# lambdaclass/AES_zero_knowledge_proof_circuit

Hardware: AMD Instinct MI355X
Metric: AES-ECB blocks proven/sec (Marlin), proof verifies (higher is better)
Workload: dtype u32 limbs (253-bit Fr / 377-bit Fq modular integers)

## Files before the change

aes_zero_knowledge_proof_circuit_amd/csrc/ff28.cuh:

```cuda
#pragma once
#include "ff.cuh"

namespace zk {

template <class P>
struct Fp28 {
    static constexpr int N = 14;
    static constexpr uint32_t MASK = (1u << 28) - 1;
    uint32_t l[N];

    ZK_HD static constexpr uint32_t mod28(int i) {
        int bit = 28 * i, w = bit >> 5, sh = bit & 31;
        uint64_t two = (w < P::N ? (uint64_t)P::mod(w) : 0) | ((w + 1 < P::N ? (uint64_t)P::mod(w + 1) : 0) << 32);
        return (uint32_t)(two >> sh) & MASK;
    }
    static constexpr uint32_t PINV = P::INV & MASK;

    ZK_HD static Fp28 zero() { Fp28 r; for (int i = 0; i < N; i++) r.l[i] = 0; return r; }
    ZK_HD bool limbs_zero() const { uint32_t o = 0; for (int i = 0; i < N; i++) o |= l[i]; return o == 0; }
    ZK_HD static bool product_is_zero(const Fp28 &v) {
        if (v.l[0] != 0u && v.l[0] != mod28(0)) return false;
        uint32_t z0 = 0, zp = 0;
#pragma unroll
        for (int i = 0; i < N; i++) { z0 |= v.l[i]; zp |= v.l[i] ^ mod28(i); }
        return z0 == 0 || zp == 0;
    }

    ZK_HD static Fp28 split(const uint32_t *w) {
        Fp28 r;
#pragma unroll
        for (int i = 0; i < N; i++) {
            int bit = 28 * i, k = bit >> 5, sh = bit & 31;
            uint64_t two = (k < P::N ? (uint64_t)w[k] : 0) | ((k + 1 < P::N ? (uint64_t)w[k + 1] : 0) << 32);
            r.l[i] = (uint32_t)(two >> sh) & MASK;
        }
        return r;
    }
    ZK_HD void pack(uint32_t *w) const {
#pragma unroll
        for (int k = 0; k < P::N; k++) {
            int bit = 32 * k, i = bit / 28, sh = bit % 28;
            uint64_t v = (uint64_t)l[i] >> sh;
            int have = 28 - sh;
            if (i + 1 < N) v |= (uint64_t)l[i + 1] << have;
            if (have + 28 < 32 && i + 2 < N) v |= (uint64_t)l[i + 2] << (have + 28);
            w[k] = (uint32_t)v;
        }
    }
    ZK_HD static Fp28 normalize(const int64_t *t) {
        Fp28 r;
        int64_t c = 0;
#pragma unroll
        for (int i = 0; i < N - 1; i++) { int64_t v = t[i] + c; r.l[i] = (uint32_t)v & MASK; c = v >> 28; }
        r.l[N - 1] = (uint32_t)(t[N - 1] + c);
        return r;
    }
    ZK_HD Fp28 operator+(const Fp28 &b) const {
        Fp28 r;
        uint32_t c = 0;
#pragma unroll
        for (int i = 0; i < N - 1; i++) { uint32_t v = l[i] + b.l[i] + c; r.l[i] = v & MASK; c = v >> 28; }
        r.l[N - 1] = l[N - 1] + b.l[N - 1] + c;
        return r;
    }
    ZK_HD Fp28 dbl() const { return *this + *this; }
    ZK_HD Fp28 add_lazy(const Fp28 &b) const { Fp28 r; for (int i = 0; i < N; i++) r.l[i] = l[i] + b.l[i]; return r; }
    ZK_HD Fp28 dbl_lazy() const { Fp28 r; for (int i = 0; i < N; i++) r.l[i] = l[i] << 1; return r; }
    template <int K> ZK_HD Fp28 sub_lazy(const Fp28 &b) const {
        Fp28 r;
#pragma unroll
        for (int i = 0; i < N; i++) {
#if defined(__HIP_DEVICE_COMPILE__)
            if (i < N - 1) { asm("v_sad_u32 %0, %1, %2, %3" : "=v"(r.l[i]) : "s"(kp_spread<K>(i)), "v"(b.l[i]), "v"(l[i])); continue; }
#endif
            r.l[i] = l[i] + kp_spread<K>(i) - b.l[i];
        }
        return r;
    }
    template <int K> ZK_HD static constexpr uint32_t kp_limb(int i) {
        uint64_t c = 0, v = 0;
        for (int j = 0; j <= i; j++) { v = (uint64_t)K * mod28(j) + c; c = v >> 28; }
        return i == N - 1 ? (uint32_t)v : (uint32_t)v & MASK;
    }
    template <int K> ZK_HD static constexpr uint32_t kp_spread(int i) {
        return i == 0 ? kp_limb<K>(0) + (1u << 28) : (i == N - 1 ? kp_limb<K>(i) - 1u : kp_limb<K>(i) + MASK);
    }
    template <int K>
    ZK_HD Fp28 sub(const Fp28 &b) const {
        Fp28 r;
        uint32_t c = 0;
#pragma unroll
        for (int i = 0; i < N - 1; i++) { uint32_t v = l[i] + kp_spread<K>(i) - b.l[i] + c; r.l[i] = v & MASK; c = v >> 28; }
        r.l[N - 1] = l[N - 1] + kp_spread<K>(N - 1) - b.l[N - 1] + c;
        return r;
    }

    ZK_HD static void reduce_row(uint64_t *t, int i) {
        if constexpr (mod28(0) == 1u && PINV == MASK) {
            const uint64_t u = t[i] + MASK;
            const uint32_t m = ~(uint32_t)u & MASK;
#pragma unroll
            for (int j = 1; j < N; j++) t[i + j] += (uint64_t)m * mod28(j);
            t[i + 1] += u >> 28;
        } else {
            uint32_t m = (((uint32_t)t[i] & MASK) * PINV) & MASK;
#pragma unroll
            for (int j = 0; j < N; j++) t[i + j] += (uint64_t)m * mod28(j);
            t[i + 1] += t[i] >> 28;
        }
    }

    ZK_HD Fp28 operator*(const Fp28 &b) const {
        uint64_t t[2 * N];
#pragma unroll
        for (int i = 0; i < 2 * N; i++) t[i] = 0;
#pragma unroll
        for (int i = 0; i < N; i++) {
#pragma unroll
            for (int j = 0; j < N; j++) t[i + j] += (uint64_t)l[j] * b.l[i];
            reduce_row(t, i);
        }
        Fp28 r;
        uint64_t c = 0;
#pragma unroll
        for (int i = 0; i < N - 1; i++) { uint64_t v = t[N + i] + c; r.l[i] = (uint32_t)v & MASK; c = v >> 28; }
        r.l[N - 1] = (uint32_t)(t[2 * N - 1] + c);
        return r;
    }
    ZK_HD static Fp28 mul_biased(const Fp28 &a, const Fp28 &b, uint64_t bias) {
        static_assert(mod28(0) == 1u && PINV == MASK, "written for p = 1 (mod 2^28)");
        uint64_t t[2 * N];
#pragma unroll
        for (int i = 0; i < 2 * N; i++) t[i] = i < N ? bias : 0;
#pragma unroll
        for (int i = 0; i < N; i++) {
#pragma unroll
            for (int j = 0; j < N; j++) t[i + j] += (uint64_t)a.l[j] * b.l[i];
            const uint64_t u = t[i];
            const uint32_t m = ~(uint32_t)u & MASK;
#pragma unroll
            for (int j = 1; j < N; j++) t[i + j] += (uint64_t)m * mod28(j);
            t[i + 1] += u >> 28;
        }
        Fp28 r;
        uint64_t c = 0;
#pragma unroll
        for (int i = 0; i < N - 1; i++) { uint64_t v = t[N + i] + c; r.l[i] = (uint32_t)v & MASK; c = v >> 28; }
        r.l[N - 1] = (uint32_t)(t[2 * N - 1] + c);
        return r;
    }
    ZK_HD static uint64_t hot_loop_bias() {
        uint64_t v = MASK;
#if defined(__HIP_DEVICE_COMPILE__)
        asm volatile("" : "+s"(v));
#endif
        return v;
    }
    ZK_HD static Fp28 fma2(const Fp28 &a, const Fp28 &b, const Fp28 &c, const Fp28 &d) {
        uint64_t t[2 * N];
#pragma unroll
        for (int i = 0; i < 2 * N; i++) t[i] = 0;
#pragma unroll
        for (int i = 0; i < N; i++) {
#pragma unroll
            for (int j = 0; j < N; j++) t[i + j] += (uint64_t)a.l[j] * b.l[i];
#pragma unroll
            for (int j = 0; j < N; j++) t[i + j] += (uint64_t)c.l[j] * d.l[i];
            reduce_row(t, i);
        }
        Fp28 r;
        uint64_t cy = 0;
#pragma unroll
        for (int i = 0; i < N - 1; i++) { uint64_t v = t[N + i] + cy; r.l[i] = (uint32_t)v & MASK; cy = v >> 28; }
        r.l[N - 1] = (uint32_t)(t[2 * N - 1] + cy);
        return r;
    }
    ZK_HD Fp28 sqr() const {
        uint64_t t[2 * N];
#pragma unroll
        for (int i = 0; i < 2 * N; i++) t[i] = 0;
        uint32_t d[N];
#pragma unroll
        for (int i = 0; i < N; i++) d[i] = l[i] << 1;
#pragma unroll
        for (int i = 0; i < N; i++) {
            t[2 * i] += (uint64_t)l[i] * l[i];
#pragma unroll
            for (int j = i + 1; j < N; j++) t[i + j] += (uint64_t)d[i] * l[j];
        }
#pragma unroll
        for (int i = 0; i < N; i++) {
            reduce_row(t, i);
        }
        Fp28 r;
        uint64_t c = 0;
#pragma unroll
        for (int i = 0; i < N - 1; i++) { uint64_t v = t[N + i] + c; r.l[i] = (uint32_t)v & MASK; c = v >> 28; }
        r.l[N - 1] = (uint32_t)(t[2 * N - 1] + c);
        return r;
    }

    ZK_HD Fp28 canonical() const {
        Fp28 v = *this;
#pragma unroll
        for (int k = 5; k >= 0; k--) {
            int64_t c = 0;
            uint32_t tl[N];
#pragma unroll
            for (int i = 0; i < N - 1; i++) { int64_t x = (int64_t)v.l[i] - ((int64_t)mod28(i) << k) + c; tl[i] = (uint32_t)x & MASK; c = x >> 28; }
            int64_t top = (int64_t)v.l[N - 1] - ((int64_t)mod28(N - 1) << k) + c;
            if (top >= 0) {
#pragma unroll
                for (int i = 0; i < N - 1; i++) v.l[i] = tl[i];
                v.l[N - 1] = (uint32_t)top;
            }
        }
        return v;
    }
    ZK_HD bool is_zero_mod_p() const { return canonical().limbs_zero(); }

    ZK_HD static Fp28 from_std(const Fp<P> &a) {
        Fp28 s = split(a.l);
        return s * k_2_400();
    }
    ZK_HD Fp<P> to_std() const {
        Fp28 y = (*this * k_2_384()).canonical();
        Fp<P> r;
        y.pack(r.l);
        return r;
    }
    ZK_HD static Fp28 k_2_384() { Fp<P> o = Fp<P>::one(); return split(o.l); }
    ZK_HD static Fp28 k_one() { return k_2_392(); }
    ZK_HD static Fp28 k_2_392() {
        Fp<P> v = Fp<P>::one();
        for (int i = 0; i < 8; i++) v = v.dbl();
        return split(v.l);
    }
    ZK_HD static Fp28 k_2_400() {
        Fp<P> v = Fp<P>::one();
        for (int i = 0; i < 16; i++) v = v.dbl();
        return split(v.l);
    }
};

using Fq377x28 = Fp28<Fq377P>;
using Fq381x28 = Fp28<Fq381P>;

}
```

aes_zero_knowledge_proof_circuit_amd/csrc/te28.cuh:

```cuda
#pragma once
#include "ec28.cuh"

namespace zk {

template <class P>
struct alignas(64) Niels28 { FpMsm<P> ymx, ypx, td; uint32_t pad[6]; };
template <class P>
struct AccTE { FpMsm<P> x, y, z, t; };

struct Te377 {
    using P = Fq377P;
    using G = Fp28<P>;
    using F = Fp<P>;
    ZK_HD static G lit28(const uint32_t (&t)[14]) { G r; for (int i = 0; i < 14; i++) r.l[i] = t[i]; return r; }
    ZK_HD static F lit(const uint32_t (&t)[12]) { F r; for (int i = 0; i < 12; i++) r.l[i] = t[i]; return r; }
    ZK_HD static F s_std() { constexpr uint32_t t[12] = FQ377_TE_S_INIT; return lit(t); }
    ZK_HD static F f_std() { constexpr uint32_t t[12] = FQ377_TE_F_INIT; return lit(t); }
    ZK_HD static F k2d_std() { constexpr uint32_t t[12] = FQ377_TE_K2D_INIT; return lit(t); }
    ZK_HD static G k2d() { constexpr uint32_t t[14] = FQ377_TE_K2D_28_INIT; return lit28(t); }
    ZK_HD static G si() { constexpr uint32_t t[14] = FQ377_TE_SI_28_INIT; return lit28(t); }
    ZK_HD static G sif() { constexpr uint32_t t[14] = FQ377_TE_SIF_28_INIT; return lit28(t); }
};

template <class P>
ZK_HD AccTE<P> te_identity() { AccTE<P> r; r.x = FpMsm<P>::zero(); r.t = r.x; r.y = FpMsm<P>::k_one(); r.z = r.y; return r; }
template <class P>
ZK_HD Niels28<P> niels_identity() { Niels28<P> r; r.ymx = FpMsm<P>::k_one(); r.ypx = r.ymx; r.td = FpMsm<P>::zero(); return r; }
template <class P>
ZK_HD Niels28<P> niels_neg(const Niels28<P> &n) { Niels28<P> r; r.ymx = n.ypx; r.ypx = n.ymx; r.td = FpMsm<P>::zero().template sub<2>(n.td); return r; }

template <class P>
ZK_HD void te_madd(AccTE<P> &a, const Niels28<P> &n) {
    using G = FpMsm<P>;
    G A = a.y.template sub_lazy<3>(a.x) * n.ymx;
    G B = a.y.add_lazy(a.x) * n.ypx;
    G C = a.t * n.td;
    G D = a.z.dbl_lazy();
    G E = B.template sub<2>(A), H = B.add_lazy(A);
    G F = D.template sub_lazy<2>(C), Gg = D + C;
    a.x = E * F; a.y = Gg * H; a.t = E * H; a.z = F * Gg;
}
template <class P>
ZK_HD Niels28<P> niels_load_signed(const Niels28<P> *rec, bool neg) {
    const FpMsm<P> *f = &rec->ymx;
    Niels28<P> r;
    r.ymx = f[neg ? 1 : 0]; r.ypx = f[neg ? 0 : 1]; r.td = rec->td;
    return r;
}
template <class P>
ZK_HD void te_madd_hot(AccTE<P> &a, Niels28<P> &n, bool neg, const Niels28<P> *next, bool next_neg, uint64_t bias) {
    using G = FpMsm<P>;
    G A = G::mul_biased(a.y.template sub_lazy<3>(a.x), n.ymx, bias);
    G B = G::mul_biased(a.y.add_lazy(a.x), n.ypx, bias);
    G C = G::mul_biased(a.t, n.td, bias);
#if defined(__HIP_DEVICE_COMPILE__)
    asm volatile("" : "+v"(A.l[G::N - 1]), "+v"(B.l[G::N - 1]), "+v"(C.l[G::N - 1]) : : "memory");
#endif
    n = niels_load_signed<P>(next, next_neg);
#if defined(__HIP_DEVICE_COMPILE__)
    asm volatile("" : "+v"(A.l[0]), "+v"(C.l[0]) : : "memory");
#endif
    G E = B.template sub_lazy<2>(A), H = B.add_lazy(A);
    G D = a.z.dbl_lazy();
    G U = D.template sub_lazy<2>(C), V = D.add_lazy(C), F, Gg;
#pragma unroll
    for (int i = 0; i < G::N; i++) { F.l[i] = neg ? V.l[i] : U.l[i]; Gg.l[i] = neg ? U.l[i] : V.l[i]; }
    a.x = G::mul_biased(E, F, bias); a.y = G::mul_biased(Gg, H, bias); a.t = G::mul_biased(E, H, bias); a.z = G::mul_biased(F, Gg, bias);
}
template <class P>
ZK_HD void te_add_inline(AccTE<P> &a, const AccTE<P> &b) {
    using G = FpMsm<P>;
    G A = a.y.template sub<3>(a.x) * b.y.template sub<3>(b.x);
    G B = (a.y + a.x) * (b.y + b.x);
    G C = (a.t * b.t) * Te377::k2d();
    G D = (a.z * b.z).dbl();
    G E = B.template sub<2>(A), H = B + A;
    G F = D.template sub<2>(C), Gg = D + C;
    a.x = E * F; a.y = Gg * H; a.t = E * H; a.z = F * Gg;
}
template <class P>
ZK_EC_FN void te_add(AccTE<P> &a, const AccTE<P> &b) { te_add_inline<P>(a, b); }
template <class P>
ZK_EC_FN void te_dbl(AccTE<P> &a) {
    using G = FpMsm<P>;
    G A = a.x.sqr(), B = a.y.sqr(), C = a.z.sqr().dbl();
    G S = (a.x + a.y).sqr(), AB = A + B;
    G E = S.template sub<3>(AB);
    G Gg = B.template sub<2>(A);
    G F = Gg.template sub<3>(C);
    G H = G::zero().template sub<3>(AB);
    a.x = E * F; a.y = Gg * H; a.t = E * H; a.z = F * Gg;
}
template <class P>
ZK_HD AccTE<P> te_neg(const AccTE<P> &a) {
    AccTE<P> r = a;
    if (!a.x.limbs_zero()) r.x = FpMsm<P>::zero().template sub<2>(a.x);
    if (!a.t.limbs_zero()) r.t = FpMsm<P>::zero().template sub<2>(a.t);
    return r;
}

template <class P>
ZK_HD XYZZ<Fp<P>> te_to_std_point(const AccTE<P> &a) {
    using G = FpMsm<P>;
    G zmy = a.z.template sub<3>(a.y), zpy = a.z + a.y;
    G xz = a.x * zmy;
    G zz = xz.sqr();
    if (zz.is_zero_mod_p()) return XYZZ<Fp<P>>::inf();
    G numx = (Te377::si() * zpy).template sub<6>(zmy);
    XYZZ<Fp<P>> o;
    o.x = ((numx * a.x) * xz).to_std();
    o.y = (((Te377::sif() * a.z) * zpy) * zz).to_std();
    o.zz = zz.to_std();
    o.zzz = (zz * xz).to_std();
    return o;
}

struct TeMapParts { Fp<Fq377P> u, v, den; };
ZK_HD TeMapParts te_map_parts(const Affine<Fp<Fq377P>> &p) {
    using F = Fp<Fq377P>;
    TeMapParts m;
    F s = Te377::s_std();
    m.u = s * (p.x + F::one());
    m.v = s * p.y;
    m.den = m.v * (m.u + F::one());
    return m;
}
ZK_HD Niels28<Fq377P> te_niels_finish(const TeMapParts &m, const Fp<Fq377P> &den_inv) {
    using F = Fp<Fq377P>;
    using G = FpMsm<Fq377P>;
    F xe = Te377::f_std() * m.u * (m.u + F::one()) * den_inv;
    F ye = (m.u - F::one()) * m.v * den_inv;
    Niels28<Fq377P> n;
    n.ymx = G::from_std(ye - xe);
    n.ypx = G::from_std(ye + xe);
    n.td = G::from_std(Te377::k2d_std() * xe * ye);
    return n;
}
ZK_HD Niels28<Fq377P> niels_from_weierstrass(const Affine<Fp<Fq377P>> &p, bool *bad) {
    if (p.is_inf()) return niels_identity<Fq377P>();
    TeMapParts m = te_map_parts(p);
    if (m.den.is_zero()) { if (bad) *bad = true; return niels_identity<Fq377P>(); }
    return te_niels_finish(m, m.den.inverse());
}

#if defined(__HIPCC__)
template <int CTRL> __device__ __forceinline__ uint32_t quad_dpp(uint32_t v) {
#if defined(__HIP_DEVICE_COMPILE__)
    return (uint32_t)__builtin_amdgcn_mov_dpp((int)v, CTRL, 0xf, 0xf, true);
#else
    return v;
#endif
}
template <int CTRL, class G> __device__ __forceinline__ G quad_move(const G &v) {
    G r;
#pragma unroll
    for (int i = 0; i < G::N; i++) r.l[i] = quad_dpp<CTRL>(v.l[i]);
    return r;
}
constexpr int QP_LANE0 = 0x00, QP_LANE1 = 0x55, QP_LANE2 = 0xAA, QP_LANE3 = 0xFF, QP_SWAP_PAIRS = 0xB1;
template <class G> __device__ __forceinline__ G quad_pick(int q, const G &v0, const G &v1, const G &v2, const G &v3) {
    G r;
#pragma unroll
    for (int i = 0; i < G::N; i++) r.l[i] = q == 0 ? v0.l[i] : (q == 1 ? v1.l[i] : (q == 2 ? v2.l[i] : v3.l[i]));
    return r;
}
template <class P>
__device__ __forceinline__ FpMsm<P> te_quad_finish(int q, const FpMsm<P> &E, const FpMsm<P> &F, const FpMsm<P> &Gg, const FpMsm<P> &H) {
    return quad_pick(q, E, Gg, F, E) * quad_pick(q, F, H, Gg, H);
}
template <class P>
__device__ __forceinline__ FpMsm<P> te_add_quad(const FpMsm<P> &a, const FpMsm<P> &b, int q) {
    using G = FpMsm<P>;
    const G oa = quad_move<QP_SWAP_PAIRS>(a), ob = quad_move<QP_SWAP_PAIRS>(b);
    const G u = quad_pick(q, oa.template sub<3>(a), a + oa, a, a), v = quad_pick(q, ob.template sub<3>(b), b + ob, b, b);
    G m = u * v;
    const G mk = m * Te377::k2d();
    m = quad_pick(q, m, m, m, mk);
    const G A = quad_move<QP_LANE0>(m), B = quad_move<QP_LANE1>(m), D = quad_move<QP_LANE2>(m).dbl(), C = quad_move<QP_LANE3>(m);
    return te_quad_finish<P>(q, B.template sub<2>(A), D.template sub<2>(C), D + C, B + A);
}
template <class P>
__device__ __forceinline__ FpMsm<P> te_dbl_quad(const FpMsm<P> &a, int q) {
    using G = FpMsm<P>;
    const G X = quad_move<QP_LANE0>(a), Y = quad_move<QP_LANE1>(a);
    const G m = quad_pick(q, a, a, a, X + Y).sqr();
    const G A = quad_move<QP_LANE0>(m), B = quad_move<QP_LANE1>(m), C = quad_move<QP_LANE2>(m).dbl(), S = quad_move<QP_LANE3>(m);
    const G AB = A + B, Gg = B.template sub<2>(A);
    return te_quad_finish<P>(q, S.template sub<3>(AB), Gg.template sub<3>(C), Gg, G::zero().template sub<3>(AB));
}
template <class P>
__device__ __forceinline__ FpMsm<P> te_identity_quad(int q) { return (q == 1 || q == 2) ? FpMsm<P>::k_one() : FpMsm<P>::zero(); }
#endif

template <class A> struct PtOps;
template <class P> struct PtOps<Acc28<P>> {
    using Params = P;
    ZK_HD static Acc28<P> identity() { return inf28<P>(); }
    ZK_HD static void add(Acc28<P> &a, const Acc28<P> &b) { add28<P>(a, b); }
    ZK_HD static void add_inline(Acc28<P> &a, const Acc28<P> &b) { add28<P>(a, b); }
    ZK_HD static void dbl(Acc28<P> &a) { dbl28<P>(a); }
    ZK_HD static Acc28<P> neg(const Acc28<P> &a) { return neg28<P>(a); }
    ZK_HD static XYZZ<Fp<P>> to_std(const Acc28<P> &a) { return to_std_point<P>(a); }
};
template <class P> struct PtOps<AccTE<P>> {
    using Params = P;
    ZK_HD static AccTE<P> identity() { return te_identity<P>(); }
    ZK_HD static void add(AccTE<P> &a, const AccTE<P> &b) { te_add<P>(a, b); }
    ZK_HD static void add_inline(AccTE<P> &a, const AccTE<P> &b) { te_add_inline<P>(a, b); }
    ZK_HD static void dbl(AccTE<P> &a) { te_dbl<P>(a); }
    ZK_HD static AccTE<P> neg(const AccTE<P> &a) { return te_neg<P>(a); }
    ZK_HD static XYZZ<Fp<P>> to_std(const AccTE<P> &a) { return te_to_std_point<P>(a); }
};

}
```

Measured before the change: 95.44.

## Split Montgomery multiply into low/high halves and interleave multiplies in TE madd

Montgomery multiplication is split into a low phase, which computes the reduction multipliers and a carry, and a product-scanning high phase that builds the upper limbs column by column. In the hot twisted-Edwards mixed-add, the three and four independent multiplies run their low phases first, then share one interleaved high phase, pinned with asm barriers and a sched_barrier. The aim is more instruction-level parallelism and fewer 64-bit accumulators live at once, since the high half no longer keeps a full 2N-word array. The cost is holding several Low structs (N multipliers each) at the same time, which may raise register pressure and lower occupancy.

```diff
diff --git a/aes_zero_knowledge_proof_circuit_amd/csrc/ff28.cuh b/aes_zero_knowledge_proof_circuit_amd/csrc/ff28.cuh
--- a/aes_zero_knowledge_proof_circuit_amd/csrc/ff28.cuh
+++ b/aes_zero_knowledge_proof_circuit_amd/csrc/ff28.cuh
@@ -127,26 +127,66 @@
         r.l[N - 1] = (uint32_t)(t[2 * N - 1] + c);
         return r;
     }
+
+    struct Low { uint32_t m[N]; uint64_t carry; };
+    template <bool ZIPPED> ZK_HD static void pin(uint64_t &acc) {
+#if defined(__HIP_DEVICE_COMPILE__)
+        if constexpr (ZIPPED) asm volatile("" : "+v"(acc)); else asm("" : "+v"(acc));
+#else
+        (void)acc;
+#endif
+    }
+    ZK_HD static Low mul_low(const Fp28 &a, const Fp28 &b, uint64_t bias) {
+        static_assert(mod28(0) == 1u && PINV == MASK, "written for p = 1 (mod 2^28)");
+        uint64_t t[N];
+        Low lo;
+#pragma unroll
+        for (int i = 0; i < N; i++) t[i] = bias;
+#pragma unroll
+        for (int i = 0; i < N; i++) {
+#pragma unroll
+            for (int j = 0; i + j < N; j++) t[i + j] += (uint64_t)a.l[j] * b.l[i];
+            const uint64_t u = t[i];
+            lo.m[i] = ~(uint32_t)u & MASK;
+#pragma unroll
+            for (int j = 1; i + j < N; j++) t[i + j] += (uint64_t)lo.m[i] * mod28(j);
+            if (i + 1 < N) t[i + 1] += u >> 28; else lo.carry = u >> 28;
+        }
+        return lo;
+    }
+    template <int W>
+    ZK_HD static void mul_high(const Fp28 *const (&a)[W], const Fp28 *const (&b)[W], const Low (&lo)[W], Fp28 *const (&r)[W]) {
+        uint64_t carry[W];
+#if defined(__HIP_DEVICE_COMPILE__)
+        if constexpr (W > 1) __builtin_amdgcn_sched_barrier(0);
+#endif
+#pragma unroll
+        for (int w = 0; w < W; w++) carry[w] = lo[w].carry;
+#pragma unroll
+        for (int k = N; k < 2 * N - 1; k++) {
+            uint64_t acc[W];
+#pragma unroll
+            for (int w = 0; w < W; w++) acc[w] = carry[w];
+#pragma unroll
+            for (int i = k - N + 1; i < N; i++) {
+#pragma unroll
+                for (int w = 0; w < W; w++) {
+                    acc[w] += (uint64_t)a[w]->l[k - i] * b[w]->l[i]; pin<(W > 1)>(acc[w]);
+                    acc[w] += (uint64_t)lo[w].m[i] * mod28(k - i); pin<(W > 1)>(acc[w]);
+                }
+            }
+#pragma unroll
+            for (int w = 0; w < W; w++) { r[w]->l[k - N] = (uint32_t)acc[w] & MASK; carry[w] = acc[w] >> 28; }
+        }
+#pragma unroll
+        for (int w = 0; w < W; w++) r[w]->l[N - 1] = (uint32_t)carry[w];
+    }
     ZK_HD static Fp28 mul_biased(const Fp28 &a, const Fp28 &b, uint64_t bias) {
-        static_assert(mod28(0) == 1u && PINV == MASK, "written for p = 1 (mod 2^28)");
-        uint64_t t[2 * N];
-#pragma unroll
-        for (int i = 0; i < 2 * N; i++) t[i] = i < N ? bias : 0;
-#pragma unroll
-        for (int i = 0; i < N; i++) {
-#pragma unroll
-            for (int j = 0; j < N; j++) t[i + j] += (uint64_t)a.l[j] * b.l[i];
-            const uint64_t u = t[i];
-            const uint32_t m = ~(uint32_t)u & MASK;
-#pragma unroll
-            for (int j = 1; j < N; j++) t[i + j] += (uint64_t)m * mod28(j);
-            t[i + 1] += u >> 28;
-        }
-        Fp28 r;
-        uint64_t c = 0;
-#pragma unroll
-        for (int i = 0; i < N - 1; i++) { uint64_t v = t[N + i] + c; r.l[i] = (uint32_t)v & MASK; c = v >> 28; }
-        r.l[N - 1] = (uint32_t)(t[2 * N - 1] + c);
+        Fp28 r;
+        const Low lo[1] = {mul_low(a, b, bias)};
+        const Fp28 *const pa[1] = {&a}, *const pb[1] = {&b};
+        Fp28 *const pr[1] = {&r};
+        mul_high<1>(pa, pb, lo, pr);
         return r;
     }
     ZK_HD static uint64_t hot_loop_bias() {
diff --git a/aes_zero_knowledge_proof_circuit_amd/csrc/te28.cuh b/aes_zero_knowledge_proof_circuit_amd/csrc/te28.cuh
--- a/aes_zero_knowledge_proof_circuit_amd/csrc/te28.cuh
+++ b/aes_zero_knowledge_proof_circuit_amd/csrc/te28.cuh
@@ -50,9 +50,15 @@
 template <class P>
 ZK_HD void te_madd_hot(AccTE<P> &a, Niels28<P> &n, bool neg, const Niels28<P> *next, bool next_neg, uint64_t bias) {
     using G = FpMsm<P>;
-    G A = G::mul_biased(a.y.template sub_lazy<3>(a.x), n.ymx, bias);
-    G B = G::mul_biased(a.y.add_lazy(a.x), n.ypx, bias);
-    G C = G::mul_biased(a.t, n.td, bias);
+    using Low = typename G::Low;
+    G A, B, C;
+    {
+        const G ymx = a.y.template sub_lazy<3>(a.x), ypx = a.y.add_lazy(a.x);
+        const Low lo[3] = {G::mul_low(ymx, n.ymx, bias), G::mul_low(ypx, n.ypx, bias), G::mul_low(a.t, n.td, bias)};
+        const G *const pa[3] = {&ymx, &ypx, &a.t}, *const pb[3] = {&n.ymx, &n.ypx, &n.td};
+        G *const pr[3] = {&A, &B, &C};
+        G::template mul_high<3>(pa, pb, lo, pr);
+    }
 #if defined(__HIP_DEVICE_COMPILE__)
     asm volatile("" : "+v"(A.l[G::N - 1]), "+v"(B.l[G::N - 1]), "+v"(C.l[G::N - 1]) : : "memory");
 #endif
@@ -65,7 +71,12 @@
     G U = D.template sub_lazy<2>(C), V = D.add_lazy(C), F, Gg;
 #pragma unroll
     for (int i = 0; i < G::N; i++) { F.l[i] = neg ? V.l[i] : U.l[i]; Gg.l[i] = neg ? U.l[i] : V.l[i]; }
-    a.x = G::mul_biased(E, F, bias); a.y = G::mul_biased(Gg, H, bias); a.t = G::mul_biased(E, H, bias); a.z = G::mul_biased(F, Gg, bias);
+    {
+        const Low lo[4] = {G::mul_low(E, F, bias), G::mul_low(Gg, H, bias), G::mul_low(E, H, bias), G::mul_low(F, Gg, bias)};
+        const G *const pa[4] = {&E, &Gg, &E, &F}, *const pb[4] = {&F, &H, &H, &Gg};
+        G *const pr[4] = {&a.x, &a.y, &a.t, &a.z};
+        G::template mul_high<4>(pa, pb, lo, pr);
+    }
 }
 template <class P>
 ZK_HD void te_add_inline(AccTE<P> &a, const AccTE<P> &b) {
```

Result: faster. 97.19, median of 6 (+1.8%).
